# InternetMaximalism/intmax-zkp-core

Hardware: NVIDIA B200
Metric: LDE+Merkle commit cells/s (higher is better)
Workload: dtype u64 (Goldilocks field, 32-bit IMAD/IADD3 limbs)

## Files before the change

### intmax_zkp_core_b200/csrc/ntt_ct_kernels.cuh

```cuda
#pragma once
#include "goldilocks.cuh"

#ifndef B200ZKP_HOST_EMU
#include <cuda.h>
#endif

namespace ntc {

using gl::u32;
using gl::u64;

static constexpr int TILE = 2048;
static constexpr int THREADS = 256;
static constexpr int MIN_BITS = 5, MAX_BITS = 8;
static constexpr int MAX_LOOP_BLOCKS = 8;
static constexpr int MAX_SRC = 8;

enum Kind : int {
    KIND_STRIDED = 0,
    KIND_STRIDED_LOOP = 1,
    KIND_FINAL_INPLACE = 2,
    KIND_FINAL_NATURAL = 3,
    KIND_PULL_LOOP = 4,
};

struct PassParams {
    const u64* in;
    u64* out;
    u64 in_col_stride, out_col_stride;
    u64 in_blk_stride, out_blk_stride;
    u32 ncols, n_blk;
    u32 n_log;
    u32 S;
    u32 C_log;
    const u64* ztab;
    u64 ztab_blk_stride;
    u64 a_scale;
    u32 use_tma;
    u32 col_run, col_period, col0, col_limit, col_sel, col_src;
    const u64* src[MAX_SRC];
    u64* copy_out;
    u64 copy_col_stride;
};

GL_FN u32 map_column(const PassParams& p, u32 v, u32& q, u32& i) {
    if (p.col_run == 0) { q = 0; i = v; return v; }
    u32 phys;
    if (p.col_sel) phys = p.col0 + (v / p.col_run) * p.col_period + p.col_src * p.col_run + v % p.col_run;
    else phys = p.col0 + v;
    const u32 in_grp = phys % p.col_period;
    q = in_grp / p.col_run;
    i = (phys / p.col_period) * p.col_run + in_grp % p.col_run;
    return phys < p.col_limit ? phys : 0xFFFFFFFFu;
}

GL_FN u32 ulog2(u32 e) {
#ifdef B200ZKP_HOST_EMU
    u32 r = 0; while (e >>= 1) r++; return r;
#else
    return 31u - (u32)__clz((int)e);
#endif
}
GL_FN u32 bitrev_bits(u32 x, u32 bits) { return bits ? (gl::brev32(x) >> (32 - bits)) : 0; }

GL_FN u64 z_index(u64 prefix, u32 e) {
    const u32 u = ulog2(e);
    return (prefix << u) + (e ^ (1u << u));
}

GL_FN void butterfly(u64& a, u64& b, u64 z) {
    const u64 t = gl::canon_cc(gl::mul_nc(b, z));
    const u64 a0 = a;
    a = gl::add_nc(a0, t);
    b = gl::sub_nc(a0, t);
}

template <int A, bool SCALE>
GL_FN void ct_group(u64 (&x)[1 << A], const u64* __restrict__ tw, u32 u0, u32 gh, u64 a_scale) {
#pragma unroll
    for (int v = 0; v < A; v++) {
        const int half = (1 << A) >> (v + 1);
        u64 z[1 << (A - 1)];
#pragma unroll
        for (int q = 0; q < (1 << v); q++) z[q] = tw[(1u << (u0 + v)) + (gh << v) + q];
#pragma unroll
        for (int j = 0; j < (1 << A); j++) {
            if (j & half) continue;
            if (SCALE && v == A - 1) x[j] = gl::canon_cc(gl::mul_nc(x[j], a_scale));
            butterfly(x[j], x[j + half], z[j >> (A - v)]);
        }
    }
}

#ifdef B200ZKP_HOST_EMU
#define NTC_FOR_THREADS(tid) for (u32 tid = 0; tid < (u32)THREADS; tid++)
#define NTC_SYNC() do {} while (0)
#else
#define NTC_FOR_THREADS(tid) for (u32 tid = threadIdx.x, once__ = 1; once__; once__ = 0)
#define NTC_SYNC() __syncthreads()
#endif

template <int A, bool SCALE>
GL_FN void run_round(const u64* __restrict__ src, u64* __restrict__ dst, const u64* __restrict__ tw, u32 tw_pitch, u32 B,
                     u32 T_log, u32 pitch, u32 u0, u64 a_scale, u32 tid) {
    const u32 st_log = B - u0 - A;
    constexpr int UNITS = 8 >> A;
#pragma unroll
    for (int r = 0; r < UNITS; r++) {
        const u32 U = tid + r * THREADS;
        const u32 t = U & ((1u << T_log) - 1), w = U >> T_log;
        const u32 gl_ = w & ((1u << st_log) - 1), gh = w >> st_log;
        const u32 gbase = (gh << (st_log + A)) + gl_;
        u64 x[1 << A];
#pragma unroll
        for (int j = 0; j < (1 << A); j++) x[j] = src[(gbase + ((u32)j << st_log)) * pitch + t];
        ct_group<A, SCALE>(x, tw + t * tw_pitch, u0, gh, a_scale);
#pragma unroll
        for (int j = 0; j < (1 << A); j++) dst[(gbase + ((u32)j << st_log)) * pitch + t] = x[j];
    }
}

template <int B, bool SCALE>
GL_FN void run_rounds(const u64* first_src, u64* tile, const u64* tw, u32 tw_pitch, u32 T_log, u32 pitch, u64 a_scale) {
    u32 u0 = 0;
    const u64* src = first_src;
    if (B % 3 == 2) { NTC_FOR_THREADS(tid) { run_round<2, false>(src, tile, tw, tw_pitch, B, T_log, pitch, u0, a_scale, tid); } u0 += 2; src = tile; NTC_SYNC(); }
    if (B % 3 == 1) { NTC_FOR_THREADS(tid) { run_round<1, false>(src, tile, tw, tw_pitch, B, T_log, pitch, u0, a_scale, tid); } u0 += 1; src = tile; NTC_SYNC(); }
#pragma unroll 1
    for (int r = 0; r < B / 3 - 1; r++) {
        NTC_FOR_THREADS(tid) { run_round<3, false>(src, tile, tw, tw_pitch, B, T_log, pitch, u0, a_scale, tid); }
        u0 += 3; src = tile;
        NTC_SYNC();
    }
    NTC_FOR_THREADS(tid) { run_round<3, SCALE>(src, tile, tw, tw_pitch, B, T_log, pitch, u0, a_scale, tid); }
}

#ifndef B200ZKP_HOST_EMU
__device__ __forceinline__ u32 smem_u32(const void* p) { return (u32)__cvta_generic_to_shared(p); }
__device__ __forceinline__ void mbar_init(u64* bar, u32 count) {
    asm volatile("mbarrier.init.shared::cta.b64 [%0], %1;" ::"r"(smem_u32(bar)), "r"(count) : "memory");
}
__device__ __forceinline__ void fence_barrier_init() { asm volatile("fence.mbarrier_init.release.cluster;" ::: "memory"); }
__device__ __forceinline__ void fence_proxy_async() { asm volatile("fence.proxy.async.shared::cta;" ::: "memory"); }
__device__ __forceinline__ void mbar_expect_tx(u64* bar, u32 bytes) {
    asm volatile("mbarrier.arrive.expect_tx.shared::cta.b64 _, [%0], %1;" ::"r"(smem_u32(bar)), "r"(bytes) : "memory");
}
__device__ __forceinline__ void mbar_wait(u64* bar, u32 parity) {
    asm volatile(
        "{\n\t.reg .pred p;\n\t"
        "NTC_WAIT:\n\t"
        "mbarrier.try_wait.parity.shared::cta.b64 p, [%0], %1;\n\t"
        "@p bra NTC_DONE;\n\t"
        "bra NTC_WAIT;\n\t"
        "NTC_DONE:\n\t}" ::"r"(smem_u32(bar)), "r"(parity) : "memory");
}
__device__ __forceinline__ void tma_load_tile(void* dst, const CUtensorMap* map, u32 c0, u32 a, u32 blk, u32 col, u64* bar) {
    asm volatile("cp.async.bulk.tensor.5d.shared::cluster.global.mbarrier::complete_tx::bytes [%0], [%1, {%2, %3, %4, %5, %6}], [%7];"
                 ::"r"(smem_u32(dst)), "l"(map), "r"(c0), "r"(0u), "r"(a), "r"(blk), "r"(col), "r"(smem_u32(bar)) : "memory");
}
__device__ __forceinline__ void tma_store_tile(const CUtensorMap* map, u32 c0, u32 a, u32 blk, u32 col, const void* src) {
    asm volatile("cp.async.bulk.tensor.5d.global.shared::cta.bulk_group [%0, {%1, %2, %3, %4, %5}], [%6];"
                 ::"l"(map), "r"(c0), "r"(0u), "r"(a), "r"(blk), "r"(col), "r"(smem_u32(src)) : "memory");
}
__device__ __forceinline__ void bulk_load(void* dst, const void* src, u32 bytes, u64* bar) {
    asm volatile("cp.async.bulk.shared::cluster.global.mbarrier::complete_tx::bytes [%0], [%1], %2, [%3];"
                 ::"r"(smem_u32(dst)), "l"(src), "r"(bytes), "r"(smem_u32(bar)) : "memory");
}
__device__ __forceinline__ void tma_commit() { asm volatile("cp.async.bulk.commit_group;" ::: "memory"); }
template <int N>
__device__ __forceinline__ void tma_wait_read() { asm volatile("cp.async.bulk.wait_group.read %0;" ::"n"(N) : "memory"); }
template <int N>
__device__ __forceinline__ void tma_wait_all() { asm volatile("cp.async.bulk.wait_group %0;" ::"n"(N) : "memory"); }
#endif

template <int B, bool LOOP>
struct StridedSmem {
    static constexpr u32 NPTS = 1u << B;
    static constexpr u32 tiles = LOOP ? 3 : 1;
    static constexpr u32 sw_words = (LOOP ? (u32)MAX_LOOP_BLOCKS : 1u) * NPTS;
    static constexpr u32 bytes = tiles * TILE * 8 + sw_words * 8 + 16;
};

template <int B, bool LOOP, typename TMap, bool PULL = false>
GL_FN void strided_body(const PassParams& p, const TMap* tm_in, const TMap* tm_out, u64* smem, u32 bid, const TMap* tm_copy = nullptr) {
    static_assert(!PULL || LOOP, "a pull pass stages its tile apart from the work tiles");
    constexpr u32 NPTS = 1u << B;
    constexpr u32 T_log = 11 - B, T = 1u << T_log;
    constexpr u32 IT = TILE / THREADS;
    u64* const stage = smem;
    u64* const work0 = LOOP ? smem + TILE : smem;
    u64* const sw = smem + StridedSmem<B, LOOP>::tiles * TILE;
    u64* const bar = sw + StridedSmem<B, LOOP>::sw_words;

    const u32 V = LOOP ? p.ncols : p.ncols * p.n_blk;
    const u32 vcol = bid % V, tile_i = bid / V;
    u32 src_q, src_i;
    const u32 col = map_column(p, LOOP ? vcol : vcol / p.n_blk, src_q, src_i);
    if (col == 0xFFFFFFFFu) return;
    const u32 in_col = PULL ? src_i : col;
    const u32 blk_fixed = LOOP ? 0u : vcol % p.n_blk;
    const u32 tiles_per_a_log = p.C_log - T_log;
    const u32 a = tile_i >> tiles_per_a_log;
    const u32 c0 = (tile_i & ((1u << tiles_per_a_log) - 1)) << T_log;
    const u64 prefix = ((u64)1 << p.S) + a;
    const u64 elem0 = ((u64)a << (B + p.C_log)) + c0;
    const u64* __restrict__ in = (PULL ? p.src[src_q] : p.in) + (u64)in_col * p.in_col_stride + (u64)blk_fixed * p.in_blk_stride + elem0;
    (void)tm_in; (void)tm_out; (void)tm_copy; (void)bar;

#ifndef B200ZKP_HOST_EMU
    const bool tma = p.use_tma != 0;
    if (tma) {
        if (threadIdx.x == 0) { mbar_init(bar, 1); fence_barrier_init(); }
        __syncthreads();
        if (threadIdx.x == 0) {
            mbar_expect_tx(bar, TILE * 8);
            tma_load_tile(stage, PULL ? tm_in + src_q : tm_in, c0, a, blk_fixed, in_col, bar);
        }
    }
#else
    const bool tma = false;
#endif
    NTC_FOR_THREADS(tid) {
        const u32 nb = LOOP ? p.n_blk : 1u;
        for (u32 i = tid; i < nb * NPTS; i += THREADS) {
            const u32 b = LOOP ? i >> B : blk_fixed, e = i & (NPTS - 1);
            if (e) sw[i] = gl::ldg(p.ztab + (u64)b * p.ztab_blk_stride + z_index(prefix, e));
        }
        if (!tma) {
            u64 v[IT];
#pragma unroll
            for (u32 it = 0; it < IT; it++) {
                const u32 i = tid + it * THREADS;
                v[it] = in[((u64)(i >> T_log) << p.C_log) + (i & (T - 1))];
            }
#pragma unroll
            for (u32 it = 0; it < IT; it++) stage[tid + it * THREADS] = v[it];
            if (PULL) {
                u64* __restrict__ cp = p.copy_out + (u64)col * p.copy_col_stride + elem0;
#pragma unroll
                for (u32 it = 0; it < IT; it++) {
                    const u32 i = tid + it * THREADS;
                    cp[((u64)(i >> T_log) << p.C_log) + (i & (T - 1))] = v[it];
                }
            }
        }
    }
#ifndef B200ZKP_HOST_EMU
    if (tma) {
        mbar_wait(bar, 0);
        if (PULL && threadIdx.x == 0) { tma_store_tile(tm_copy, c0, a, 0, col, stage); tma_commit(); }
    }
#endif
    NTC_SYNC();

    const u32 n_loop = LOOP ? p.n_blk : 1u;
    for (u32 lb = 0; lb < n_loop; lb++) {
        const u32 blk = LOOP ? lb : blk_fixed;
        u64* const tile = LOOP ? work0 + (lb & 1) * TILE : work0;
#ifndef B200ZKP_HOST_EMU
        if (LOOP && tma && lb >= 2) { if (threadIdx.x == 0) tma_wait_read<1>(); __syncthreads(); }
#endif
        run_rounds<B, false>(LOOP ? stage : tile, tile, sw + (LOOP ? lb * NPTS : 0), 0, T_log, T, 0);
        u64* __restrict__ out = p.out + (u64)col * p.out_col_stride + (u64)blk * p.out_blk_stride + elem0;
#ifndef B200ZKP_HOST_EMU
        if (tma) {
            fence_proxy_async();
            __syncthreads();
            if (threadIdx.x == 0) { tma_store_tile(tm_out, c0, a, blk, col, tile); tma_commit(); }
            continue;
        }
#endif
        NTC_SYNC();
        NTC_FOR_THREADS(tid) {
#pragma unroll
            for (u32 it = 0; it < IT; it++) {
                const u32 i = tid + it * THREADS;
                out[((u64)(i >> T_log) << p.C_log) + (i & (T - 1))] = tile[i];
            }
        }
        NTC_SYNC();
    }
#ifndef B200ZKP_HOST_EMU
    if (tma && threadIdx.x == 0) tma_wait_read<0>();
#endif
}

template <int B>
struct FinalSmem {
    static constexpr u32 NPTS = 1u << B, T = (u32)TILE >> B;
    static constexpr u32 TP = T + 1, TWP = NPTS + 1;
    static constexpr u32 tw_words = T * TWP;
    static constexpr u32 bytes = (NPTS * TP + tw_words) * 8 + 16;
};

template <int B, bool NATURAL>
GL_FN void final_body(const PassParams& p, u64* smem, u32 bid) {
    constexpr u32 NPTS = 1u << B;
    constexpr u32 T_log = 11 - B, T = 1u << T_log, TP = FinalSmem<B>::TP, TWP = FinalSmem<B>::TWP;
    constexpr u32 IT = TILE / THREADS;
    u64* const tile = smem;
    u64* const swb = smem + NPTS * TP;
    u64* const bar = swb + FinalSmem<B>::tw_words;
    (void)bar;
    const u32 batches_log = p.n_log - B;
    const u32 V = p.ncols * p.n_blk;
    const u32 vcol = bid % V, tile_i = bid / V;
    u32 src_q, src_i;
    const u32 col = map_column(p, vcol / p.n_blk, src_q, src_i), blk = vcol % p.n_blk;
    if (col == 0xFFFFFFFFu) return;
    const u32 batch0 = tile_i << T_log;
    const u64* __restrict__ in = p.in + (u64)col * p.in_col_stride + (u64)blk * p.in_blk_stride;
    u64* __restrict__ out = p.out + (u64)col * p.out_col_stride + (u64)blk * p.out_blk_stride;
    const u64* __restrict__ ztile = p.ztab + (u64)blk * p.ztab_blk_stride + (u64)tile_i * FinalSmem<B>::tw_words;

#ifndef B200ZKP_HOST_EMU
    if (threadIdx.x == 0) { mbar_init(bar, 1); fence_barrier_init(); }
    __syncthreads();
    if (threadIdx.x == 0) {
        mbar_expect_tx(bar, FinalSmem<B>::tw_words * 8);
        bulk_load(swb, ztile, FinalSmem<B>::tw_words * 8, bar);
    }
#else
    for (u32 i = 0; i < FinalSmem<B>::tw_words; i++) swb[i] = ztile[i];
#endif
    NTC_FOR_THREADS(tid) {
        u64 v[IT];
#pragma unroll
        for (u32 it = 0; it < IT; it += 2) {
            const u32 i = 2 * (tid + (it / 2) * THREADS);
            const u32 b = i >> B, g = i & (NPTS - 1);
            const u32 a_b = NATURAL ? bitrev_bits(batch0 + b, batches_log) : batch0 + b;
#ifdef B200ZKP_HOST_EMU
            v[it] = in[((u64)a_b << B) + g]; v[it + 1] = in[((u64)a_b << B) + g + 1];
#else
            const ulonglong2 q = *reinterpret_cast<const ulonglong2*>(in + ((u64)a_b << B) + g);
            v[it] = q.x; v[it + 1] = q.y;
#endif
        }
#pragma unroll
        for (u32 it = 0; it < IT; it += 2) {
            const u32 i = 2 * (tid + (it / 2) * THREADS);
            const u32 b = i >> B, g = i & (NPTS - 1);
            tile[g * TP + b] = v[it];
            tile[(g + 1) * TP + b] = v[it + 1];
        }
    }
#ifndef B200ZKP_HOST_EMU
    mbar_wait(bar, 0);
#endif
    NTC_SYNC();

    if (p.a_scale) run_rounds<B, true>(tile, tile, swb, TWP, T_log, TP, p.a_scale);
    else run_rounds<B, false>(tile, tile, swb, TWP, T_log, TP, 0);
    NTC_SYNC();

    NTC_FOR_THREADS(tid) {
        if (NATURAL) {
#pragma unroll
            for (u32 it = 0; it < IT; it++) {
                const u32 i = tid + it * THREADS;
                const u32 tau = i & (T - 1), r = i >> T_log;
                const u32 g = bitrev_bits(r, B);
                out[((u64)r << batches_log) + batch0 + tau] = gl::canon_cc(tile[g * TP + tau]);
            }
        } else {
#pragma unroll
            for (u32 it = 0; it < IT; it += 2) {
                const u32 i = 2 * (tid + (it / 2) * THREADS);
                const u32 b = i >> B, g = i & (NPTS - 1);
                const u64 x0 = gl::canon_cc(tile[g * TP + b]), x1 = gl::canon_cc(tile[(g + 1) * TP + b]);
#ifdef B200ZKP_HOST_EMU
                out[((u64)(batch0 + b) << B) + g] = x0; out[((u64)(batch0 + b) << B) + g + 1] = x1;
#else
                *reinterpret_cast<ulonglong2*>(out + ((u64)(batch0 + b) << B) + g) = make_ulonglong2(x0, x1);
#endif
            }
        }
    }
}

#ifndef B200ZKP_HOST_EMU
template <int B, int KIND>
__global__ void __launch_bounds__(THREADS, 4)
ct_pass_kernel(const PassParams p, const __grid_constant__ CUtensorMap tm_in, const __grid_constant__ CUtensorMap tm_out) {
    extern __shared__ __align__(128) unsigned char ntc_smem_raw[];
    u64* smem = reinterpret_cast<u64*>(ntc_smem_raw);
    if (KIND == KIND_STRIDED) strided_body<B, false>(p, &tm_in, &tm_out, smem, blockIdx.x);
    else if (KIND == KIND_STRIDED_LOOP) strided_body<B, true>(p, &tm_in, &tm_out, smem, blockIdx.x);
    else if (KIND == KIND_FINAL_INPLACE) final_body<B, false>(p, smem, blockIdx.x);
    else final_body<B, true>(p, smem, blockIdx.x);
}

struct PullMaps { CUtensorMap m[MAX_SRC]; };
template <int B>
struct PullSmem {
    static constexpr u32 NPTS = 1u << B;
    static constexpr u32 sw_words = (u32)MAX_LOOP_BLOCKS * NPTS;
    static constexpr u32 bytes = 4 * TILE * 8 + sw_words * 8 + 32;
};

template <int B>
__device__ __forceinline__ void pull_decode(const PassParams& p, u32 bid, u32& col, u32& in_col, u32& q, u32& a, u32& c0) {
    constexpr u32 T_log = 11 - B;
    const u32 vcol = bid % p.ncols, tile_i = bid / p.ncols;
    u32 i;
    col = map_column(p, vcol, q, i);
    in_col = i;
    const u32 tiles_per_a_log = p.C_log - T_log;
    a = tile_i >> tiles_per_a_log;
    c0 = (tile_i & ((1u << tiles_per_a_log) - 1)) << T_log;
}

template <int B>
__global__ void __launch_bounds__(THREADS, 4)
ct_pull_kernel(const PassParams p, const __grid_constant__ PullMaps tm_src, const __grid_constant__ CUtensorMap tm_out,
               const __grid_constant__ CUtensorMap tm_copy, const u32 total) {
    extern __shared__ __align__(128) unsigned char ntc_smem_raw[];
    u64* const smem = reinterpret_cast<u64*>(ntc_smem_raw);
    if (!p.use_tma) {
        for (u32 bid = blockIdx.x; bid < total; bid += gridDim.x) {
            strided_body<B, true, CUtensorMap, true>(p, tm_src.m, &tm_out, smem, bid, &tm_copy);
            __syncthreads();
        }
        return;
    }
    constexpr u32 NPTS = 1u << B;
    constexpr u32 T_log = 11 - B, T = 1u << T_log;
    u64* const stage0 = smem;
    u64* const work0 = smem + 2 * TILE;
    u64* const sw = smem + 4 * TILE;
    u64* const bar = sw + PullSmem<B>::sw_words;
    if (blockIdx.x >= total) return;
    if (threadIdx.x == 0) { mbar_init(bar, 1); mbar_init(bar + 1, 1); fence_barrier_init(); }
    __syncthreads();
    u32 col, in_col, q, a, c0;
    if (threadIdx.x == 0) {
        pull_decode<B>(p, blockIdx.x, col, in_col, q, a, c0);
        mbar_expect_tx(bar, TILE * 8);
        tma_load_tile(stage0, &tm_src.m[q], c0, a, 0, in_col, bar);
    }
    u32 it = 0;
    for (u32 bid = blockIdx.x; bid < total; bid += gridDim.x, it++) {
        const u32 slot = it & 1;
        u64* const stage = stage0 + slot * TILE;
        if (threadIdx.x == 0 && bid + gridDim.x < total) {
            pull_decode<B>(p, bid + gridDim.x, col, in_col, q, a, c0);
            mbar_expect_tx(bar + (slot ^ 1), TILE * 8);
            tma_load_tile(stage0 + (slot ^ 1) * TILE, &tm_src.m[q], c0, a, 0, in_col, bar + (slot ^ 1));
        }
        pull_decode<B>(p, bid, col, in_col, q, a, c0);
        const u64 prefix = ((u64)1 << p.S) + a;
        for (u32 i = threadIdx.x; i < p.n_blk * NPTS; i += THREADS) {
            const u32 b = i >> B, e = i & (NPTS - 1);
            if (e) sw[i] = gl::ldg(p.ztab + (u64)b * p.ztab_blk_stride + z_index(prefix, e));
        }
        mbar_wait(bar + slot, (it >> 1) & 1);
        if (threadIdx.x == 0) { tma_store_tile(&tm_copy, c0, a, 0, col, stage); tma_commit(); }
        __syncthreads();
        for (u32 lb = 0; lb < p.n_blk; lb++) {
            u64* const tile = work0 + (lb & 1) * TILE;
            if (lb >= 2) { if (threadIdx.x == 0) tma_wait_read<1>(); __syncthreads(); }
            run_rounds<B, false>(stage, tile, sw + lb * NPTS, 0, T_log, T, 0);
            fence_proxy_async();
            __syncthreads();
            if (threadIdx.x == 0) { tma_store_tile(&tm_out, c0, a, lb, col, tile); tma_commit(); }
        }
        if (threadIdx.x == 0) tma_wait_read<0>();
        __syncthreads();
    }
}

__device__ __forceinline__ u64 z_entry(u64 i, u32 n_log, const u64* __restrict__ spow, const u64* __restrict__ lo,
                                       const u64* __restrict__ hi, u32 lo_bits, u64 last_scale) {
    if (!i) return 0;
    const u32 l = 63u - (u32)__clzll((long long)i);
    const u32 j = (u32)(i - ((u64)1 << l));
    const u64 e = (u64)bitrev_bits(j, l) << (n_log - 1 - l);
    const u64 w = gl::mul(gl::ldg(lo + (e & (((u64)1 << lo_bits) - 1))), gl::ldg(hi + (e >> lo_bits)));
    u64 r = gl::mul(w, gl::ldg(spow + (n_log - 1 - l)));
    if (last_scale && l == n_log - 1) r = gl::mul(r, last_scale);
    return r;
}
__global__ void build_ztab_kernel(u64* __restrict__ out, u64 count, u32 n_log, const u64* __restrict__ spow, const u64* __restrict__ lo,
                                  const u64* __restrict__ hi, u32 lo_bits, u64 last_scale) {
    const u64 i = (u64)blockIdx.x * blockDim.x + threadIdx.x;
    if (i >= count) return;
    out[(u64)blockIdx.y * count + i] = z_entry(i, n_log, spow + (u64)blockIdx.y * n_log, lo, hi, lo_bits, last_scale);
}
__global__ void build_zfinal_kernel(u64* __restrict__ out, u64 words, u32 n_log, u32 B, u32 natural, const u64* __restrict__ spow,
                                    const u64* __restrict__ lo, const u64* __restrict__ hi, u32 lo_bits, u64 last_scale) {
    const u64 x = (u64)blockIdx.x * blockDim.x + threadIdx.x;
    if (x >= words) return;
    const u32 T_log = 11 - B, TWP = (1u << B) + 1, S = n_log - B;
    const u64 tile_i = x / ((u64)TWP << T_log);
    const u32 rem = (u32)(x - tile_i * ((u64)TWP << T_log));
    const u32 b = rem / TWP, e = rem - b * TWP;
    u64 r = 0;
    if (e >= 1 && e < (1u << B)) {
        const u32 batch = (u32)(tile_i << T_log) + b;
        const u32 a_b = natural ? bitrev_bits(batch, S) : batch;
        r = z_entry(z_index(((u64)1 << S) + a_b, e), n_log, spow + (u64)blockIdx.y * n_log, lo, hi, lo_bits, last_scale);
    }
    out[(u64)blockIdx.y * words + x] = r;
}
#endif

}
```

Measured before the change: 1.097 billion.

## Hand-code butterfly canon/add in PTX, pack twiddle smem, cap registers

Replaces the butterfly's canonicalisation and modular add with inline PTX carry-chain sequences that use a constant-memory zero operand, so the compiler cannot fold the carry logic. Packs the per-block twiddle table in shared memory by dropping the unused index-0 slot, which shrinks the footprint. Replaces launch_bounds with per-kind __maxnreg__ caps to force higher occupancy. The register caps risk spills, and the PTX tricks depend on how the compiler schedules them.

```diff
diff --git a/intmax_zkp_core_b200/csrc/ntt_ct_kernels.cuh b/intmax_zkp_core_b200/csrc/ntt_ct_kernels.cuh
--- a/intmax_zkp_core_b200/csrc/ntt_ct_kernels.cuh
+++ b/intmax_zkp_core_b200/csrc/ntt_ct_kernels.cuh
@@ -68,10 +68,48 @@
     return (prefix << u) + (e ^ (1u << u));
 }
 
+#ifdef B200ZKP_HOST_EMU
+GL_FN u64 bf_canon(u64 a) { return gl::canon_cc(a); }
+GL_FN u64 bf_add(u64 a, u64 c) { return gl::add_nc(a, c); }
+#else
+static __device__ __constant__ u32 NTC_ZERO = 0;
+GL_FN u64 bf_canon(u64 a) {
+    u64 r;
+    asm("{\n\t"
+        ".reg .u32 l0, l1, s0, s1, m, h;\n\t"
+        ".reg .pred q;\n\t"
+        "mov.b64 {l0, l1}, %1;\n\t"
+        "add.cc.u32 s0, l0, 0xFFFFFFFF;\n\t"
+        "addc.cc.u32 s1, l1, 0;\n\t"
+        "madc.lo.u32 h, %2, %2, l1;\n\t"
+        "addc.u32 m, 0, 0;\n\t"
+        "setp.ne.u32 q, m, 0;\n\t"
+        "selp.u32 l0, s0, l0, q;\n\t"
+        "mov.b64 %0, {l0, h};\n\t"
+        "}" : "=l"(r) : "l"(a), "r"(NTC_ZERO));
+    return r;
+}
+GL_FN u64 bf_add(u64 a, u64 c) {
+    u64 r;
+    asm("{\n\t"
+        ".reg .u32 l0, l1, m;\n\t"
+        ".reg .u64 t;\n\t"
+        "add.cc.u64 t, %1, %2;\n\t"
+        "madc.lo.u32 m, %3, %3, 0;\n\t"
+        "mov.b64 {l0, l1}, t;\n\t"
+        "sub.cc.u32 l0, l0, m;\n\t"
+        "subc.u32 l1, l1, 0;\n\t"
+        "add.u32 l1, l1, m;\n\t"
+        "mov.b64 %0, {l0, l1};\n\t"
+        "}" : "=l"(r) : "l"(a), "l"(c), "r"(NTC_ZERO));
+    return r;
+}
+#endif
+
 GL_FN void butterfly(u64& a, u64& b, u64 z) {
-    const u64 t = gl::canon_cc(gl::mul_nc(b, z));
+    const u64 t = bf_canon(gl::mul_nc(b, z));
     const u64 a0 = a;
-    a = gl::add_nc(a0, t);
+    a = bf_add(a0, t);
     b = gl::sub_nc(a0, t);
 }
 
@@ -177,7 +215,7 @@
 struct StridedSmem {
     static constexpr u32 NPTS = 1u << B;
     static constexpr u32 tiles = LOOP ? 3 : 1;
-    static constexpr u32 sw_words = (LOOP ? (u32)MAX_LOOP_BLOCKS : 1u) * NPTS;
+    static constexpr u32 sw_words = (LOOP ? (u32)MAX_LOOP_BLOCKS : 1u) * (NPTS - 1);
     static constexpr u32 bytes = tiles * TILE * 8 + sw_words * 8 + 16;
 };
 
@@ -224,7 +262,7 @@
         const u32 nb = LOOP ? p.n_blk : 1u;
         for (u32 i = tid; i < nb * NPTS; i += THREADS) {
             const u32 b = LOOP ? i >> B : blk_fixed, e = i & (NPTS - 1);
-            if (e) sw[i] = gl::ldg(p.ztab + (u64)b * p.ztab_blk_stride + z_index(prefix, e));
+            if (e) sw[i - (i >> B) - 1] = gl::ldg(p.ztab + (u64)b * p.ztab_blk_stride + z_index(prefix, e));
         }
         if (!tma) {
             u64 v[IT];
@@ -260,7 +298,7 @@
 #ifndef B200ZKP_HOST_EMU
         if (LOOP && tma && lb >= 2) { if (threadIdx.x == 0) tma_wait_read<1>(); __syncthreads(); }
 #endif
-        run_rounds<B, false>(LOOP ? stage : tile, tile, sw + (LOOP ? lb * NPTS : 0), 0, T_log, T, 0);
+        run_rounds<B, false>(LOOP ? stage : tile, tile, sw + (LOOP ? lb * (NPTS - 1) : 0) - 1, 0, T_log, T, 0);
         u64* __restrict__ out = p.out + (u64)col * p.out_col_stride + (u64)blk * p.out_blk_stride + elem0;
 #ifndef B200ZKP_HOST_EMU
         if (tma) {
@@ -381,7 +419,7 @@
 
 #ifndef B200ZKP_HOST_EMU
 template <int B, int KIND>
-__global__ void __launch_bounds__(THREADS, 4)
+__global__ void __maxnreg__(KIND == KIND_STRIDED_LOOP ? 56 : 40)
 ct_pass_kernel(const PassParams p, const __grid_constant__ CUtensorMap tm_in, const __grid_constant__ CUtensorMap tm_out) {
     extern __shared__ __align__(128) unsigned char ntc_smem_raw[];
     u64* smem = reinterpret_cast<u64*>(ntc_smem_raw);
```

New measurement: 1.109 billion, median of 6. 1.01x the previous value.
